# mihikamd/DP-GSAT

Hardware: AMD Instinct MI355X
Metric: million edges/s (attn+sample+aggregate fwd+bwd) (higher is better)
Workload: dtype f32

## Files before the change

dp_gsat_amd/_lib.py:

```python
from __future__ import annotations

import ctypes
import os
from ctypes import c_char_p, c_float, c_int, c_int32, c_int64, c_size_t, c_uint64, c_void_p

import torch

_HERE = os.path.dirname(os.path.abspath(__file__))
LIB_PATH = os.path.join(_HERE, "libgsat_hip.so")

P, I64, I32, F32, SZ, INT, U64 = c_void_p, c_int64, c_int32, c_float, c_size_t, c_int, c_uint64

SIGNATURES = {
    "gsat_abi_version": (INT, []),
    "gsat_seed_next": (INT, [P, P, P]),
    "gsat_last_error": (c_char_p, []),
    "gsat_csr_workspace_bytes": (SZ, [I64, I64]),
    "gsat_rev_workspace_bytes": (SZ, [I64]),
    "gsat_build_csr": (INT, [P, P, I64, I64, P, P, P, P, P, SZ, P]),
    "gsat_reverse_edge_perm": (INT, [P, I64, I64, P, P, P, SZ, P]),
    "gsat_reverse_edge_perm_csr": (INT, [P, P, P, P, P, P, P, P, I64, I64, P, P, P]),
    "gsat_segment_ptr": (INT, [P, I64, I64, P, P, P]),
    "gsat_gather_i64": (INT, [P, I64, P, I64, P, P]),
    "gsat_row_chunks_workspace_bytes": (SZ, [I64]),
    "gsat_row_chunks": (INT, [P, I64, P, P, SZ, P]),
    "gsat_long_row_partial_floats": (SZ, [I64, I64]),
    "gsat_aggr_sum_fwd": (INT, [P, P, P, P, P, P, P, I64, I64, I64, F32, P, P, P, P]),
    "gsat_aggr_sum_bwd": (INT, [P, P, P, P, P, P, P, I64, I64, I64, F32, P, P, P, P, P, P]),
    "gsat_pna_fwd": (INT, [P, P, P, P, P, P, I64, I64, P, INT, P, INT, F32, F32, P, P]),
    "gsat_pna_bwd": (INT, [P, P, P, P, P, P, P, I64, I64, P, INT, P, INT, F32, F32, P, P, P, P, P]),
    "gsat_pna_long_row_floats": (SZ, [I64, I64, INT]),
    "gsat_pna_fwd_long": (INT, [P, P, P, P, P, P, I64, I64, I64, P, INT, P, INT, F32, F32, P, P, P, P]),
    "gsat_pna_bwd_long": (INT, [P, P, P, P, P, P, P, I64, I64, I64, P, INT, P, INT, F32, F32, P, P, P, P, P, P, P]),
    "gsat_pna_tile_plan": (INT, [I64, I64, P, P, P]),
    "gsat_pna_build_tiles": (INT, [P, P, P, P, P, I64, INT, INT, INT, P, P, P, P]),
    "gsat_pna_bwd_tiled": (INT, [P, P, P, P, P, P, P, I64, INT, INT, INT, P, P, I64, I64, I64, P, INT, P, INT, P, P, P, P, P, P, P]),
    "gsat_pna_fwd_compact": (INT, [P, P, P, P, P, I64, I64, P, INT, P, P, P]),
    "gsat_pna_post_fwd": (INT, [P, P, P, I64, I64, INT, P, I64, P, I64, P, P]),
    "gsat_pna_post_dw_workspace_floats": (SZ, [I64, I64, INT, I64]),
    "gsat_pna_post_dw": (INT, [P, P, P, I64, I64, INT, P, I64, P, P, SZ, P]),
    "gsat_pna_fwd_node_att": (INT, [P, P, P, P, I64, I64, P, INT, P, INT, F32, F32, P, P]),
    "gsat_pna_bwd_tiled_node_att": (INT, [P, P, P, P, P, P, I64, INT, INT, INT, P, P, I64, I64, I64, P, INT, P, INT, P, P, P, P, P, P, P, INT, P]),
    "gsat_csr_pair_workspace_bytes": (SZ, [I64, I64]),
    "gsat_build_csr_pair": (INT, [P, I64, I64] + [P] * 12 + [P, SZ, P]),
    "gsat_segment_ptr32": (INT, [P, I64, I64, P, P, P, P]),
    "gsat_bn_workspace_floats": (SZ, [I64, I64]),
    "gsat_bn_fwd": (INT, [P, P, P, P, P, I64, I64, INT, F32, F32, INT, P, P, P, P, P]),
    "gsat_bn_bwd": (INT, [P, P, P, P, P, P, I64, I64, INT, INT, P, P, P, P, P]),
    "gsat_bn_act_fwd": (INT, [P, P, P, P, P, I64, I64, INT, F32, F32, INT, P, F32, U64, P, P, P, P, P, P]),
    "gsat_bn_act_bwd": (INT, [P, P, P, P, P, P, I64, I64, INT, INT, F32, U64, P, P, P, P, P, P, P]),
    "gsat_bn_local_sum": (INT, [P, P, I64, I64, P, P, P]),
    "gsat_bn_apply_fwd": (INT, [P, P, P, P, P, I64, I64, INT, P, F32, U64, P, P, P]),
    "gsat_bn_local_bwd_sums": (INT, [P, P, P, P, P, P, I64, I64, INT, F32, U64, P, P, P, P, P]),
    "gsat_bn_apply_bwd": (INT, [P, P, P, P, P, P, P, P, I64, P, I64, I64, INT, F32, U64, P, P, P, P]),
    "gsat_relu_dropout_fwd": (INT, [P, I64, I64, F32, U64, P, P, P]),
    "gsat_relu_dropout_bwd": (INT, [P, P, I64, I64, F32, P, P]),
    "gsat_colsum_workspace_floats": (SZ, [I64]),
    "gsat_colsum": (INT, [P, I64, I64, P, P, P]),
    "gsat_embsum_fwd": (INT, [P, P, INT, P, I64, I64, P, P]),
    "gsat_onehot_rows": (INT, [P, P, INT, I64, I64, P, P]),
    "gsat_gemm_workspace_floats": (SZ, [INT, I64, I64, I64]),
    "gsat_gemm_f32": (INT, [INT, INT, I64, I64, I64, P, I64, P, I64, P, I64, P, INT, P, SZ, P]),
    "gsat_gemm_bf16x3": (INT, [INT, INT, I64, I64, I64, P, I64, P, I64, P, I64, P, INT, P, SZ, P]),
    "gsat_attn_fwd_workspace_bytes": (SZ, [P]),
    "gsat_attn_fwd_kind": (I32, [P]),
    "gsat_attn_bwd_workspace_bytes": (SZ, [P]),
    "gsat_attn_fwd": (INT, [P, P]),
    "gsat_attn_bwd": (INT, [P, P, P]),
# ... 94 lines not shown
```

dp_gsat_amd/csrc/bookkeeping.hip:

```cpp
#include "common.h"
#include <rocprim/rocprim.hpp>

namespace gsat {

constexpr int64_t GSAT_COUNTING_MAX_KEYS = 1 << 20;

static thread_local char g_err[512] = {0};
void set_error(const char* fmt, ...) {
    va_list ap;
    va_start(ap, fmt);
    vsnprintf(g_err, sizeof(g_err), fmt, ap);
    va_end(ap);
}
const char* get_error() { return g_err; }

__global__ void k_seed_next(uint64_t* __restrict__ state, uint64_t* __restrict__ out) {
    const uint64_t c = state[1] + 1;
    state[1] = c;
    uint64_t z = state[0] + c * 0x9E3779B97F4A7C15ull;
    z = (z ^ (z >> 30)) * 0xBF58476D1CE4E5B9ull;
    z = (z ^ (z >> 27)) * 0x94D049BB133111EBull;
    z ^= z >> 31;
    out[0] = z & 0x7FFFFFFFFFFFFFFFull;
}
// ... 298 lines not shown
            if (k >= N) {
                const int c0 = (int32_t)(first[N] >> 32);
                rowptr_src[k - N] = beg - (int32_t)E;
                chunk_ptr_src[k - N] = chunks - c0;
                if (k == 2 * N) status[2] = chunks - c0;
            }
        } else {
            rowptr_dst[k] = beg;
        }
        if (k < R && (int32_t)first[k + 1] - beg > COUNT_ELEM_ROW)
            long_rows[atomicAdd(long_count, 1)] = (int32_t)k;
    }
    if (k < total) {
        const int r = rowkey[k];
        const int beg = (int32_t)first[r], end = (int32_t)first[r + 1];
        if (end - beg > COUNT_ELEM_ROW) return;
        const int v = slot[k];
        int rank = 0;
        for (int j = beg; j < end; ++j) rank += slot[j] < v;
        perm[beg + rank] = v;
    }
}

__global__ __launch_bounds__(COUNT_LONG_BLOCK) void k_pair_order_long(const int64_t* __restrict__ first, int32_t* __restrict__ slot,
                                                                       int32_t* __restrict__ perm, const int32_t* __restrict__ long_rows,
                                                                       const int32_t* __restrict__ long_count) {
    __shared__ int32_t buf[COUNT_CHUNK];
    const int nlong = *long_count;
    for (int q = blockIdx.x; q < nlong; q += gridDim.x) {
        const int k = long_rows[q];
        const int beg = (int32_t)first[k], end = (int32_t)first[k + 1], deg = end - beg;
        const int nchunks = (deg + COUNT_CHUNK - 1) / COUNT_CHUNK;
        for (int c = 0; c < nchunks; ++c) {
            const int cb = beg + c * COUNT_CHUNK, len = min(COUNT_CHUNK, end - cb);
            int p2 = 64;
            while (p2 < len) p2 <<= 1;
            for (int i = threadIdx.x; i < p2; i += COUNT_LONG_BLOCK) buf[i] = i < len ? slot[cb + i] : 0x7fffffff;
            __syncthreads();
            for (int size = 2; size <= p2; size <<= 1)
                for (int stride = size >> 1; stride > 0; stride >>= 1) {
                    for (int t = threadIdx.x; t < (p2 >> 1); t += COUNT_LONG_BLOCK) {
                        const int lo = 2 * t - (t & (stride - 1)), hi = lo + stride;
                        const bool up = (lo & size) == 0;
                        const int a = buf[lo], b = buf[hi];
                        if ((a > b) == up) { buf[lo] = b; buf[hi] = a; }
                    }
                    __syncthreads();
                }
            int32_t* outp = nchunks == 1 ? perm : slot;
            for (int i = threadIdx.x; i < len; i += COUNT_LONG_BLOCK) outp[cb + i] = buf[i];
            __syncthreads();
        }
        if (nchunks == 1) continue;
        for (int i = threadIdx.x; i < deg; i += COUNT_LONG_BLOCK) {
            const int v = slot[beg + i], own = i / COUNT_CHUNK;
            int r = i - own * COUNT_CHUNK;
            for (int c = 0; c < nchunks; ++c) {
                if (c == own) continue;
                const int32_t* base = slot + beg + c * COUNT_CHUNK;
                int lo = 0, hi = min(COUNT_CHUNK, deg - c * COUNT_CHUNK);
                while (lo < hi) {
                    const int mid = (lo + hi) >> 1;
                    if (base[mid] < v) lo = mid + 1; else hi = mid;
                }
                r += lo;
            }
            perm[beg + r] = v;
        }
        __syncthreads();
    }
}

struct CountAndChunks {
    const int32_t* cnt;
    __host__ __device__ int64_t operator()(int k) const {
        const int deg = cnt[k];
        const int64_t chunks = deg > GSAT_LONG_ROW_EDGES ? (deg + GSAT_LONG_ROW_EDGES - 1) / GSAT_LONG_ROW_EDGES : 0;
        return (int64_t)deg + (chunks << 32);
    }
};

static size_t count_scan_items_temp_bytes(int64_t items) {
    size_t tb = 0;
    auto in = rocprim::make_transform_iterator(rocprim::make_counting_iterator<int>(0), CountAndChunks{nullptr});
    int64_t* p = nullptr;
    (void)rocprim::exclusive_scan(nullptr, tb, in, p, (int64_t)0, (size_t)std::max<int64_t>(items, 1), rocprim::plus<int64_t>(), (hipStream_t)0);
    return align_up(tb, 256) + 256;
}
static size_t count_scan_temp_bytes(int64_t n) { return count_scan_items_temp_bytes(2 * n + 1); }

static bool counting_build(int64_t E) {
    static const int on = [] { const char* e = getenv("GSAT_CSR_COUNTING"); return e ? atoi(e) : 1; }();
    return on && 2 * E <= GSAT_COUNTING_MAX_KEYS;
}

// ... 7 lines not shown
        if (r >= num_rows) return 0;
        const int deg = rp[r + 1] - rp[r];
        return deg > GSAT_LONG_ROW_EDGES ? (deg + GSAT_LONG_ROW_EDGES - 1) / GSAT_LONG_ROW_EDGES : 0;
    }
};

__global__ void k_split_chunk_ptrs(const int32_t* __restrict__ scan, int64_t N, int32_t* __restrict__ chunk_ptr_dst,
                                   int32_t* __restrict__ chunk_ptr_src, int32_t* __restrict__ status) {
    int64_t i = (int64_t)blockIdx.x * blockDim.x + threadIdx.x;
    if (i > N) return;
    const int32_t d = scan[i], s = scan[N + 1 + i] - scan[N + 1];
    chunk_ptr_dst[i] = d;
    chunk_ptr_src[i] = s;
    if (i == N) { status[1] = d; status[2] = s; }
}

static size_t chunk2_scan_temp_bytes(int64_t n) {
    size_t tb = 0;
    auto in = rocprim::make_transform_iterator(rocprim::make_counting_iterator<int>(0), ChunkCount2{nullptr, nullptr, 0});
    int32_t* out = nullptr;
    (void)rocprim::exclusive_scan(nullptr, tb, in, out, 0, (size_t)(2 * n + 2), rocprim::plus<int>(), (hipStream_t)0);
    return align_up(tb, 256) + 256;
}

template <class K>
static size_t sort_temp_bytes(int64_t n) {
    size_t tb = 0;
    K* k = nullptr;
    int32_t* v = nullptr;
    (void)rocprim::radix_sort_pairs(nullptr, tb, k, k, v, v, (size_t)(n > 0 ? n : 1), 0, (unsigned)(8 * sizeof(K)), (hipStream_t)0);
    return align_up(tb, 256) + 256;
}

}

using namespace gsat;

extern "C" {

int gsat_abi_version(void) { return GSAT_ABI_VERSION; }

int gsat_seed_next(uint64_t* state, uint64_t* out, void* stream) {
    GSAT_REQUIRE(state && out, GSAT_ERR_ARG, "gsat_seed_next: null pointer");
    gsat::k_seed_next<<<1, 1, 0, (hipStream_t)stream>>>(state, out);
    GSAT_LAUNCH_CHECK();
    return GSAT_OK;
// ... 171 lines not shown
        GSAT_LAUNCH_CHECK();
        k_pair_order_long<<<256, COUNT_LONG_BLOCK, 0, stream>>>(first, slot, perm, long_rows, cnt + 2 * N + 1);
        GSAT_LAUNCH_CHECK();
    } else {
        GSAT_CHECK_HIP(gsat::zero_async(err_flag, 4 * sizeof(int32_t), stream));
        k_make_pair_keys<<<ceil_div(E, B), B, 0, stream>>>(edge_index, E, N, keys_in, ids, src32, dst32, err_flag);
        GSAT_LAUNCH_CHECK();
        const int end_bit = bits_for((uint64_t)(2 * N - 1));
        GSAT_CHECK_HIP(rocprim::radix_sort_pairs(temp, tb, keys_in, keys_out, ids, perm, (size_t)(2 * E), 0, (unsigned)end_bit, stream));
        k_pair_rowptrs<<<ceil_div(2 * N + 2, B), B, 0, stream>>>(keys_out, E, N, rowptr_dst, rowptr_src);
        GSAT_LAUNCH_CHECK();
    }
    k_pair_gather<<<ceil_div(2 * E, B), B, 0, stream>>>(edge_index, perm, E, N, rowptr_dst, src_by_dst, eid_by_dst, dst_by_src, eid_by_src,
                                                        slot_dst_of_srcslot);
    GSAT_LAUNCH_CHECK();
    if (counting) return GSAT_OK;
    auto in = rocprim::make_transform_iterator(rocprim::make_counting_iterator<int>(0), ChunkCount2{rowptr_dst, rowptr_src, (int)N});
    GSAT_CHECK_HIP(rocprim::exclusive_scan(temp2, tc, in, scan, 0, (size_t)(2 * N + 2), rocprim::plus<int>(), stream));
    k_split_chunk_ptrs<<<ceil_div(N + 1, B), B, 0, stream>>>(scan, N, chunk_ptr_dst, chunk_ptr_src, err_flag);
    GSAT_LAUNCH_CHECK();
    return GSAT_OK;
}

size_t gsat_row_chunks_workspace_bytes(int64_t num_rows) { return chunk_scan_temp_bytes(num_rows); }

int gsat_row_chunks(const int32_t* rowptr, int64_t num_rows, int32_t* chunk_ptr, void* workspace, size_t ws_bytes, void* stream_) {
    hipStream_t stream = (hipStream_t)stream_;
    GSAT_REQUIRE(num_rows >= 0 && num_rows < (1ll << 31) - 1 && rowptr && chunk_ptr, GSAT_ERR_ARG, "gsat_row_chunks: bad argument");
    size_t tb = chunk_scan_temp_bytes(num_rows);
    GSAT_REQUIRE(workspace && ws_bytes >= tb, GSAT_ERR_WORKSPACE, "gsat_row_chunks: workspace %zu < %zu", ws_bytes, tb);
    auto in = rocprim::make_transform_iterator(rocprim::make_counting_iterator<int>(0), ChunkCount{rowptr, (int)num_rows});
    GSAT_CHECK_HIP(rocprim::exclusive_scan(workspace, tb, in, chunk_ptr, 0, (size_t)(num_rows + 1), rocprim::plus<int>(), stream));
    return GSAT_OK;
}

int gsat_segment_ptr(const int64_t* seg_ids, int64_t n, int64_t num_seg, int32_t* ptr, int32_t* flags, void* stream_) {
    hipStream_t stream = (hipStream_t)stream_;
    GSAT_REQUIRE(n >= 0 && num_seg >= 0 && ptr && flags, GSAT_ERR_ARG, "gsat_segment_ptr: bad argument");
    GSAT_REQUIRE(n < (1ll << 31), GSAT_ERR_UNSUPPORTED, "gsat_segment_ptr: >2^31 rows");
    const int B = 256;
    GSAT_CHECK_HIP(gsat::zero_async(flags, sizeof(int32_t), stream));
    if (n > 0) {
        GSAT_REQUIRE(seg_ids, GSAT_ERR_ARG, "gsat_segment_ptr: null ids");
        k_check_sorted<<<ceil_div(n, B), B, 0, stream>>>(seg_ids, n, num_seg, flags);
        GSAT_LAUNCH_CHECK();
    }
// ... 28 lines not shown
```

dp_gsat_amd/csrc/common.h:

```cpp
#pragma once
#include <cstring>
#include <cstdint>
#include <cstdio>
#include <cstdarg>
#include <hip/hip_runtime.h>

#include "../../include/gsat_hip.h"

namespace gsat {

void set_error(const char* fmt, ...);
const char* get_error();

#define GSAT_CHECK_HIP(expr)                                                                  \
    do {                                                                                      \
        hipError_t _e = (expr);                                                               \
        if (_e != hipSuccess) {                                                               \
            gsat::set_error("%s:%d: %s -> %s", __FILE__, __LINE__, #expr, hipGetErrorString(_e)); \
            return GSAT_ERR_HIP;                                                              \
        }                                                                                     \
    } while (0)

#define GSAT_REQUIRE(cond, code, ...)                                                         \
    do {                                                                                      \
// ... 102 lines not shown
        c0 = n0; c1 = n1; c2 = n2; c3 = n3;
        k0 += 0x9E3779B9u; k1 += 0xBB67AE85u;
    }
    return make_uint4(c0, c1, c2, c3);
}

__device__ __forceinline__ float philox_noise_u(uint64_t seed, int row) {
    const uint4 r = philox4x32(seed, (uint32_t)row, 0u, 4u, 0x5A17u);
    return ((float)(r.x >> 9) + 0.5f) * (1.0f / 8388608.0f);
}

struct SeedRef {
    uint64_t value;
    const uint64_t* dev;
    __device__ __forceinline__ uint64_t get() const { return dev ? *dev : value; }
};

__device__ __forceinline__ float4 philox_keep4(uint64_t seed, int layer, int row, int c, float p) {
    uint4 r = philox4x32(seed, (uint32_t)row, (uint32_t)(c >> 2), (uint32_t)layer, 0x5A17u);
    const float k = 1.0f / 16777216.0f;
    return make_float4((float)(r.x >> 8) * k >= p ? 1.f : 0.f, (float)(r.y >> 8) * k >= p ? 1.f : 0.f,
                       (float)(r.z >> 8) * k >= p ? 1.f : 0.f, (float)(r.w >> 8) * k >= p ? 1.f : 0.f);
}
#endif

}
```

dp_gsat_amd/csrc/pna.hip:

```cpp
#include "common.h"
#include "pna_math.h"

namespace gsat {

constexpr int PNA_BLOCK = 128;
constexpr int SC_AMP = GSAT_SCALE_AMPLIFICATION, SC_ATT = GSAT_SCALE_ATTENUATION, SC_LIN = GSAT_SCALE_LINEAR, SC_INVLIN = GSAT_SCALE_INVERSE_LINEAR;

struct PnaCfg {
    int A, S;
    int aggr[8];
    int scal[8];
    float avg_lin, avg_log;
};

__device__ __forceinline__ int pna_xcd_remap(int b, int nb) {
    int q = nb >> 3, r = nb & 7, x = b & 7, i = b >> 3;
    return (x < r ? x * (q + 1) : r * (q + 1) + (x - r) * q) + i;
}

__device__ __forceinline__ float scaler_factor(int s, float deg, float avg_lin, float avg_log) {
    switch (s) {
        case SC_AMP: return logf(deg + 1.f) / avg_log;
        case SC_ATT: return deg == 0.f ? 1.f : avg_log / logf(deg + 1.f);
        case SC_LIN: return deg / avg_lin;
// ... 557 lines not shown
                        de.z = fmaf(Qe.z, w * ee.z, Pe.z) + (k == emin.z ? gmn_e.z : 0.f) + (k == emax.z ? gmx_e.z : 0.f);
                        de.w = fmaf(Qe.w, w * ee.w, Pe.w) + (k == emin.w ? gmn_e.w : 0.f) + (k == emax.w ? gmx_e.w : 0.f);
                        if (dedge) st4(dedge + (size_t)e * H + c, f4scale(w, de));
                        da += f4dot(de, ee);
                    }
                }
                if (datt) {
                    da = group_sum<LPR>(da);
                    if (lane == 0) datt[e] = c0 ? datt[e] + da : da;
                }
            }
        }
    }
}

constexpr int TILE_BLOCK = 512;

__global__ void k_pna_tiles(const int32_t* __restrict__ node_ptr, const int32_t* __restrict__ node_seg, const int32_t* __restrict__ rowptr,
                            const int32_t* __restrict__ rowptr_src, int N, int TN, int slack, int T, int4* __restrict__ desc,
                            int32_t* __restrict__ spill_count) {
    const int t = blockIdx.x * blockDim.x + threadIdx.x;
    if (t == 0 && spill_count) *spill_count = 0;
    if (t > T) return;
    const int64_t p = (int64_t)t * TN;
    int start = N;
    if (t < T && p < N) {
        start = (int)p;
        if (node_seg) {
            const int g0 = node_ptr[node_seg[p]];
            start = min((int)p, max(g0, (int)p - slack));
        }
    }
    desc[t] = make_int4(start, rowptr[start], rowptr_src[start], 0);
}

template <int LPR, int NAGG, bool NATT>
__global__ __launch_bounds__(TILE_BLOCK, 4) void k_pna_bwd_tile(
    const float* __restrict__ x, const float* __restrict__ att, const float* __restrict__ dout, const int32_t* __restrict__ rowptr,
    const int32_t* __restrict__ col, const int32_t* __restrict__ eid, const int4* __restrict__ desc,
    const int32_t* __restrict__ rowptr_src, const int32_t* __restrict__ slot_map, int H, int TE, int RCAP, float* dx,
    float* __restrict__ dmsg, float* datt, float* __restrict__ dw, const float* __restrict__ dx_add, int datt_acc) {
    constexpr int GPB = LaneGroups<LPR, TILE_BLOCK>::GPB;
    constexpr int RPW = 64 / LPR;
    constexpr int NSEG = NAGG * 2;
    extern __shared__ float4 smem4[];
    float4* erow = smem4;
    int* s_col = reinterpret_cast<int*>(erow + (size_t)TE * LPR);
    int* s_eid = s_col + TE;
    float* s_w = reinterpret_cast<float*>(s_eid);
    float* s_att = reinterpret_cast<float*>(s_eid + TE);
    int* s_slot = reinterpret_cast<int*>(s_att + TE);
    int* s_rp = s_slot + TE;
    int* s_rps = s_rp + RCAP + 1;
    float* s_na = reinterpret_cast<float*>(s_rps + RCAP + 1);
    float* s_dna = s_na + RCAP + 1;
    const int tid = threadIdx.x, wave = tid >> 6;
// ... 178 lines not shown
            acc.x += r.x; acc.y += r.y; acc.z += r.z; acc.w += r.w;
        }
        float sw = 0.f;
        for (int s_ = sb; s_ < se; ++s_) {
            const int kl = s_ < nsl ? s_slot[s_] : slot_map[s0 + s_] - k0;
            if (kl >= 0 && kl < ne) {
                const float4 v = erow[(size_t)kl * LPR + lane];
                acc.x += v.x; acc.y += v.y; acc.z += v.z; acc.w += v.w;
                if (NATT) sw += s_w[kl];
            }
        }
        st4(dx + (size_t)j * H + c, acc);
        if (NATT && datt && lane == 0) datt[j] = (s_dna[j - n0] + sw) + dprev;
    }
}

__global__ void k_pna_spill_rows(const int4* __restrict__ desc, int TN, int TE, const int32_t* __restrict__ rowptr_src,
                                 const int32_t* __restrict__ slot_map, int num_rows, int32_t* __restrict__ spill_rows,
                                 int32_t* __restrict__ spill_count) {
    const int j = blockIdx.x * blockDim.x + threadIdx.x;
    if (j >= num_rows) return;
    const int sb = rowptr_src[j], se = rowptr_src[j + 1];
    if (sb == se) return;
    int t = j / TN;
    if (j >= desc[t + 1].x) ++t;
    const int k0 = desc[t].y, ne = min(desc[t + 1].y - k0, TE);
    bool flag = false;
    for (int s_ = sb; s_ < se && !flag; ++s_) {
        const int k = slot_map[s_];
        flag = k < k0 || k >= k0 + ne;
    }
    if (flag) {
        const int idx = atomicAdd(spill_count, 1);
        if (idx < num_rows) spill_rows[idx] = j;
    }
}

template <int LPR>
__global__ __launch_bounds__(256) void k_pna_bwd_spill(const float* __restrict__ dmsg, const int4* __restrict__ desc, int TN, int TE,
                                                       const int32_t* __restrict__ rowptr_src, const int32_t* __restrict__ slot_map,
                                                       const int32_t* __restrict__ spill_rows, const int32_t* __restrict__ spill_count,
                                                       int num_rows, int H, float* __restrict__ dx, const float* __restrict__ dw,
                                                       float* __restrict__ dna) {
    const LaneGroups<LPR, 256> lg;
    constexpr int GPB = LaneGroups<LPR, 256>::GPB;
    const int lane = lg.lane, c = lane * 4;
    const int count = min(*spill_count, num_rows);
    if (lg.grp < 0) return;
    for (int i = blockIdx.x * GPB + lg.grp; i < count; i += gridDim.x * GPB) {
        const int j = spill_rows[i];
        const int sb = rowptr_src[j], se = rowptr_src[j + 1];
        int t = j / TN;
        if (j >= desc[t + 1].x) ++t;
        const int k0 = desc[t].y, ne = min(desc[t + 1].y - k0, TE);
// ... 325 lines not shown
```

dp_gsat_amd/graph_index.py:

```python
from __future__ import annotations

import os
from collections import OrderedDict
from typing import Optional

import torch

from . import _lib
from ._lib import call, ptr, stream


_SYNC_FREE = False
_VALIDATED: set = set()



_HUBS_SEEN = [False]
_STATUS_RING = []


def _harvest_status():
    bad = None
    for slot in _STATUS_RING:
        host, ev, owner = slot
# ... 30 lines not shown
    slot[2] = weakref.ref(index)
    index._status_event = slot[1]


_STRICT = False


def set_strict(flag: bool) -> None:
    global _STRICT
    _STRICT = bool(flag)


def strict() -> bool:
    return _STRICT


def set_sync_free(flag: bool) -> None:
    global _SYNC_FREE
    _SYNC_FREE = bool(flag)


def sync_free() -> bool:
    return _SYNC_FREE


def _i32(n, device):
    return torch.empty(max(int(n), 1), dtype=torch.int32, device=device)[: int(n)]


class BatchIndex:
    def __init__(self, edge_index: torch.Tensor, num_nodes: int):
        if edge_index.dim() != 2 or edge_index.shape[0] != 2 or edge_index.dtype != torch.int64:
            raise ValueError("edge_index must be an int64 tensor of shape [2, E]")
        _lib.load()
        if not edge_index.is_cuda:
            raise _lib.GsatHipError("BatchIndex needs a ROCm edge_index (no CPU fallback)")
        self._key_tensor = edge_index
        self.edge_index = edge_index.contiguous()
        self.N = int(num_nodes)
        self.E = int(edge_index.shape[1])
        self.device = edge_index.device
        dev = self.device
        E, N = self.E, self.N
        pair_build = os.environ.get("GSAT_CSR_PAIR", "1") != "0"
        self._err = (torch.empty if pair_build else torch.zeros)(8, dtype=torch.int32, device=dev)
        self._err3_fresh = True
# ... 6 lines not shown
         self.dst32) = (ints[i, :E] for i in range(7))
        if os.environ.get("GSAT_CSR_PAIR", "1") == "0":
            src, dst = self.edge_index[0], self.edge_index[1]
            wb = max(call_size("gsat_csr_workspace_bytes", E, N), 256)
            w1 = torch.empty(wb, dtype=torch.uint8, device=dev)
            call("gsat_build_csr", ptr(dst), ptr(src), E, N, ptr(self.rowptr_dst), ptr(self.src_by_dst), ptr(self.eid_by_dst),
                 ptr(self._err), ptr(w1), wb, stream())
            call("gsat_build_csr", ptr(src), ptr(dst), E, N, ptr(self.rowptr_src), ptr(self.dst_by_src), ptr(self.eid_by_src),
                 ptr(self._err), ptr(w1), wb, stream())
            cb = max(call_size("gsat_row_chunks_workspace_bytes", N), 256)
            w2 = torch.empty(cb, dtype=torch.uint8, device=dev)
            call("gsat_row_chunks", ptr(self.rowptr_dst), N, ptr(self.chunk_ptr_dst), ptr(w2), cb, stream())
            call("gsat_row_chunks", ptr(self.rowptr_src), N, ptr(self.chunk_ptr_src), ptr(w2), cb, stream())
            call("gsat_narrow_i64", ptr(src), E, ptr(self.src32), stream())
            call("gsat_narrow_i64", ptr(dst), E, ptr(self.dst32), stream())
            if E:
                inv = torch.empty(E, dtype=torch.int32, device=dev)
                inv[self.eid_by_dst.long()] = torch.arange(E, dtype=torch.int32, device=dev)
                self._slot_dst_of_srcslot.copy_(inv[self.eid_by_src.long()])
            self._partials, self._long, self._tiles = {}, None, {}
            self._checked, self._rev, self._rev_dev, self._rev_flags, self._undirected, self._graphs = False, None, None, None, None, {}
            self._long_async, self._status_queued, self._status_event = None, False, None
            return
        ws_bytes = max(call_size("gsat_csr_pair_workspace_bytes", E, N), 256)
        ws = torch.empty(ws_bytes, dtype=torch.uint8, device=dev)
        call("gsat_build_csr_pair", ptr(self.edge_index), E, N, ptr(self.rowptr_dst), ptr(self.src_by_dst), ptr(self.eid_by_dst),
             ptr(self.rowptr_src), ptr(self.dst_by_src), ptr(self.eid_by_src), ptr(self._slot_dst_of_srcslot),
             ptr(self.chunk_ptr_dst), ptr(self.chunk_ptr_src), ptr(self.src32), ptr(self.dst32), ptr(self._err), ptr(ws), ws_bytes,
             stream())
        self._partials = {}
        self._tiles = {}
        self._long = None
        self._checked = False
        self._rev = None
        self._rev_dev = None
        self._rev_flags = None
        self._undirected = None
        self._graphs = {}
        self._long_async = None
        self._status_queued, self._status_event = False, None
        if _SYNC_FREE:
            self._validate_once()

    @property
    def long_rows(self):
        if _SYNC_FREE and self._long is None:
            return (self.chunk_ptr_dst, self.chunk_ptr_src) if _HUBS_SEEN[0] else (None, None)
        if self._long is None or not self._checked:
            self._readback()
        return (self.chunk_ptr_dst if self._long[0] else None, self.chunk_ptr_src if self._long[1] else None)

    @property
    def long_rows_nowait(self):
        if _STRICT and not _SYNC_FREE and not self._checked and not torch.cuda.is_current_stream_capturing():
            self._readback()
        if self._long is not None:
            known = self._long
        else:
            if not _SYNC_FREE and not torch.cuda.is_current_stream_capturing():
                if not self._status_queued:
                    self._status_queued = True
                    _queue_status(self)
                elif self._long_async is None and self._status_event is not None and self._status_event.query():
                    _harvest_status()
            known = self._long_async
# ... 78 lines not shown
            if self._undirected is None:
                self._readback()
        return self._undirected

    @property
    def rev(self) -> Optional[torch.Tensor]:
        self.is_undirected
        return self._rev

    @property
    def slot_dst_of_srcslot(self) -> torch.Tensor:
        return self._slot_dst_of_srcslot

    def pna_tiles(self, H: int):
        import ctypes
        seg = next(iter(self._graphs.values())) if self._graphs else None
        key = (int(H), id(seg))
        hit = self._tiles.get(key)
        if hit is not None:
            return hit
        if H < 64:
            self._tiles[key] = False
            return False
        nominal, slack, ecap = ctypes.c_int32(), ctypes.c_int32(), ctypes.c_int32()
        budget = int(os.environ.get("GSAT_PNA_TILE_LDS", "0"))
        if _lib.load().gsat_pna_tile_plan(int(H), budget, ctypes.byref(nominal), ctypes.byref(slack), ctypes.byref(ecap)) != 0:
            self._tiles[key] = False
            return False
        T = (self.N + nominal.value - 1) // nominal.value
        tile_ptr = torch.empty(T + 1, 4, dtype=torch.int32, device=self.device)
        spill = torch.empty(self.N + 1, dtype=torch.int32, device=self.device)
        call("gsat_pna_build_tiles", ptr(seg.node_ptr) if seg is not None else None, ptr(seg.node_seg32) if seg is not None else None,
             ptr(self.rowptr_dst), ptr(self.rowptr_src), ptr(self._slot_dst_of_srcslot) if self.E else None, self.N, nominal.value,
             slack.value, ecap.value, ptr(tile_ptr), ptr(spill[1:]), ptr(spill[:1]), stream())
        out = (tile_ptr, T, nominal.value, nominal.value + slack.value, ecap.value, spill)
        self._tiles = {key: out}
        return out

    def graphs(self, batch: torch.Tensor, num_graphs: Optional[int] = None) -> "GraphSegments":
        key = (batch.data_ptr(), batch._version, int(batch.shape[0]))
        seg = self._graphs.get(key)
        if seg is None:
            if not self._err3_fresh:
                self._err[3:4].zero_()
            self._err3_fresh = False
            seg = GraphSegments(self, batch, num_graphs)
            self._graphs = {key: seg}
            self._checked = False
            if _SYNC_FREE:
                self._validate_once()
        return seg


class GraphSegments:

    def __init__(self, index: BatchIndex, batch: torch.Tensor, num_graphs: Optional[int] = None):
        if batch.dtype != torch.int64 or batch.dim() != 1:
            raise ValueError("batch must be an int64 vector")
        self.index = index
        self.batch = batch.contiguous()
        dev = batch.device
        n = int(batch.shape[0])
        if num_graphs is None:
            num_graphs = int(batch.max().item()) + 1 if n > 0 else 0
        self.G = int(num_graphs)
        self.node_ptr = torch.empty(self.G + 1, dtype=torch.int32, device=dev)
        flags = index._err[3:4]
        self.node_seg32 = _i32(n, dev)
        call("gsat_segment_ptr32", ptr(self.batch), n, self.G, ptr(self.node_ptr), ptr(self.node_seg32), ptr(flags), stream())
        self._flags = flags
        self._edge = None

    def check(self):
        self.index._checked = False
        self.index.check()

    @property
    def edge_segments(self):
        if self._edge is None:
            ix = self.index
            E, dev = ix.E, ix.device
            eg = torch.empty(max(E, 1), dtype=torch.int64, device=dev)[:E]
            call("gsat_gather_i64", ptr(self.batch), int(self.batch.shape[0]), ptr(ix.edge_index[0].contiguous()), E, ptr(eg), stream())
            ws_bytes = max(call_size("gsat_csr_workspace_bytes", E, self.G), 256)
            ws = torch.empty(ws_bytes, dtype=torch.uint8, device=dev)
            eptr = torch.empty(self.G + 1, dtype=torch.int32, device=dev)
            order = _i32(E, dev)
            err = torch.zeros(1, dtype=torch.int32, device=dev)
            call("gsat_build_csr", ptr(eg), None, E, self.G, ptr(eptr), None, ptr(order), ptr(err), ptr(ws), ws_bytes, stream())
            eg32 = _i32(E, dev)
            call("gsat_narrow_i64", ptr(eg), E, ptr(eg32), stream())
            self._edge = (eptr, order, eg, eg32)
# ... 29 lines not shown
```

include/gsat_hip.h:

```cpp
#ifndef GSAT_HIP_H
#define GSAT_HIP_H

#include <stddef.h>
#include <stdint.h>

#ifdef __cplusplus
extern "C" {
#endif

#define GSAT_ABI_VERSION 4

#define GSAT_OK 0
#define GSAT_ERR_HIP (-1)
#define GSAT_ERR_ARG (-2)
#define GSAT_ERR_WORKSPACE (-3)
#define GSAT_ERR_UNSUPPORTED (-4)
#define GSAT_ERR_BLAS (-5)

int gsat_abi_version(void);

int gsat_seed_next(uint64_t* state, uint64_t* out, void* stream);
const char* gsat_last_error(void);


// ... 3 lines not shown
int gsat_build_csr(const int64_t* rows, const int64_t* other, int64_t num_edges, int64_t num_rows,
                   int32_t* rowptr, int32_t* other_sorted, int32_t* perm, int32_t* err_flag,
                   void* workspace, size_t workspace_bytes, void* stream);

size_t gsat_csr_pair_workspace_bytes(int64_t E, int64_t num_nodes);
int gsat_build_csr_pair(const int64_t* edge_index, int64_t E, int64_t num_nodes, int32_t* rowptr_dst, int32_t* src_by_dst,
                        int32_t* eid_by_dst, int32_t* rowptr_src, int32_t* dst_by_src, int32_t* eid_by_src,
                        int32_t* slot_dst_of_srcslot, int32_t* chunk_ptr_dst, int32_t* chunk_ptr_src, int32_t* src32,
                        int32_t* dst32, int32_t* err_flag, void* workspace, size_t workspace_bytes, void* stream);

int gsat_reverse_edge_perm(const int64_t* edge_index, int64_t num_edges, int64_t num_nodes,
                           int32_t* rev, int32_t* flags, void* workspace, size_t workspace_bytes,
                           void* stream);

int gsat_reverse_edge_perm_csr(const int32_t* src32, const int32_t* dst32, const int32_t* rowptr_dst, const int32_t* src_by_dst,
                               const int32_t* eid_by_dst, const int32_t* rowptr_src, const int32_t* dst_by_src,
                               const int32_t* eid_by_src, int64_t num_edges, int64_t num_nodes, int32_t* rev, int32_t* flags,
                               void* stream);

int gsat_segment_ptr(const int64_t* seg_ids, int64_t num_rows, int64_t num_segments, int32_t* ptr,
                     int32_t* flags, void* stream);
int gsat_segment_ptr32(const int64_t* seg_ids, int64_t n, int64_t num_segments, int32_t* ptr, int32_t* seg_ids32,
                       int32_t* flags, void* stream);

int gsat_gather_i64(const int64_t* table, int64_t table_len, const int64_t* index, int64_t n, int64_t* out, void* stream);


#define GSAT_LONG_ROW_EDGES 256
size_t gsat_row_chunks_workspace_bytes(int64_t num_rows);
int gsat_row_chunks(const int32_t* rowptr, int64_t num_rows, int32_t* chunk_ptr ,
                    void* workspace, size_t workspace_bytes, void* stream);
size_t gsat_long_row_partial_floats(int64_t num_edges, int64_t H);

int gsat_aggr_sum_fwd(const float* x, const float* self_rows, const float* att, const float* edge_emb,
                      const int32_t* rowptr, const int32_t* col, const int32_t* eid,
                      int64_t num_rows, int64_t num_edges, int64_t H, float self_coef, float* out,
                      const int32_t* chunk_ptr, float* partial, void* stream);

int gsat_aggr_sum_bwd(const float* x, const float* att, const float* edge_emb, const float* dout,
                      const int32_t* rowptr_src, const int32_t* dst_sorted, const int32_t* eid_src,
                      int64_t num_rows, int64_t num_edges, int64_t H, float self_coef, float* dx, float* datt,
                      float* dedge_emb, const int32_t* chunk_ptr, float* partial, void* stream);


#define GSAT_AGG_SUM 0
#define GSAT_AGG_MEAN 1
// ... 230 lines not shown
```

Baseline: 125.6.

## Merge CSR pair build, batch segments and PNA tile plan into one fused index build

Adds a single batch-index build entry point that folds the CSR pair construction, the batch segment pointers and the PNA tile descriptors and spill detection into fewer multi-role kernels. Index construction is deferred lazily until the batch vector is known, so everything can be built in one pass. The goal is to cut kernel launches and repeated edge passes in per-batch bookkeeping. In exchange it adds lazy attribute machinery and a global tile-width heuristic, which makes the control flow more complex.

After: 126.4, median of 6. No clear change (+0.7%).

```diff
diff --git a/dp_gsat_amd/_lib.py b/dp_gsat_amd/_lib.py
--- a/dp_gsat_amd/_lib.py
+++ b/dp_gsat_amd/_lib.py
@@ -44,6 +44,8 @@
     "gsat_csr_pair_workspace_bytes": (SZ, [I64, I64]),
     "gsat_build_csr_pair": (INT, [P, I64, I64] + [P] * 12 + [P, SZ, P]),
     "gsat_segment_ptr32": (INT, [P, I64, I64, P, P, P, P]),
+    "gsat_batch_index_workspace_bytes": (SZ, [I64, I64]),
+    "gsat_build_batch_index": (INT, [P, I64, I64] + [P] * 12 + [P, I64, I64, P, P, INT, INT, INT, P, P, P, P, SZ, P]),
     "gsat_bn_workspace_floats": (SZ, [I64, I64]),
     "gsat_bn_fwd": (INT, [P, P, P, P, P, I64, I64, INT, F32, F32, INT, P, P, P, P, P]),
     "gsat_bn_bwd": (INT, [P, P, P, P, P, P, I64, I64, INT, INT, P, P, P, P, P]),
diff --git a/dp_gsat_amd/csrc/bookkeeping.hip b/dp_gsat_amd/csrc/bookkeeping.hip
--- a/dp_gsat_amd/csrc/bookkeeping.hip
+++ b/dp_gsat_amd/csrc/bookkeeping.hip
@@ -344,12 +344,9 @@
     }
 }
 
-__global__ __launch_bounds__(COUNT_LONG_BLOCK) void k_pair_order_long(const int64_t* __restrict__ first, int32_t* __restrict__ slot,
-                                                                       int32_t* __restrict__ perm, const int32_t* __restrict__ long_rows,
-                                                                       const int32_t* __restrict__ long_count) {
-    __shared__ int32_t buf[COUNT_CHUNK];
-    const int nlong = *long_count;
-    for (int q = blockIdx.x; q < nlong; q += gridDim.x) {
+__device__ __forceinline__ void order_long_rows(const int64_t* __restrict__ first, int32_t* __restrict__ slot, int32_t* __restrict__ perm,
+                                                const int32_t* __restrict__ long_rows, int nlong, int q0, int qstride, int32_t* buf) {
+    for (int q = q0; q < nlong; q += qstride) {
         const int k = long_rows[q];
         const int beg = (int32_t)first[k], end = (int32_t)first[k + 1], deg = end - beg;
         const int nchunks = (deg + COUNT_CHUNK - 1) / COUNT_CHUNK;
@@ -393,6 +390,13 @@
     }
 }
 
+__global__ __launch_bounds__(COUNT_LONG_BLOCK) void k_pair_order_long(const int64_t* __restrict__ first, int32_t* __restrict__ slot,
+                                                                       int32_t* __restrict__ perm, const int32_t* __restrict__ long_rows,
+                                                                       const int32_t* __restrict__ long_count) {
+    __shared__ int32_t buf[COUNT_CHUNK];
+    order_long_rows(first, slot, perm, long_rows, *long_count, blockIdx.x, gridDim.x, buf);
+}
+
 struct CountAndChunks {
     const int32_t* cnt;
     __host__ __device__ int64_t operator()(int k) const {
@@ -446,6 +450,151 @@
     (void)rocprim::exclusive_scan(nullptr, tb, in, out, 0, (size_t)(2 * n + 2), rocprim::plus<int>(), (hipStream_t)0);
     return align_up(tb, 256) + 256;
 }
+
+__global__ void k_index_prep(int32_t* __restrict__ cnt, int64_t ncnt, int32_t* __restrict__ status, int32_t* __restrict__ spill_count,
+                             const int64_t* __restrict__ ids, int64_t n, int64_t num_seg, int32_t* __restrict__ ids32,
+                             int32_t* __restrict__ ptr) {
+    const int64_t i = (int64_t)blockIdx.x * blockDim.x + threadIdx.x;
+    if (i < ncnt) cnt[i] = 0;
+    if (i < 4) status[i] = 0;
+    if (i == 0 && spill_count) *spill_count = 0;
+    if (!ptr) return;
+    if (i < n) {
+        const int64_t v = ids[i];
+        ids32[i] = (int32_t)(v < 0 ? 0 : (v >= num_seg ? num_seg - 1 : v));
+    }
+    if (i <= num_seg) {
+        int64_t lo = 0, hi = n;
+        while (lo < hi) {
+            int64_t mid = (lo + hi) >> 1;
+            if (ids[mid] < i) lo = mid + 1; else hi = mid;
+        }
+        ptr[i] = (int32_t)lo;
+    }
+}
+
+__global__ void k_pair_count_check(const int64_t* __restrict__ ei, int64_t E, int64_t N, int32_t* __restrict__ cnt,
+                                   int32_t* __restrict__ src32, int32_t* __restrict__ dst32, int32_t* status,
+                                   const int64_t* __restrict__ ids, int64_t n, int64_t num_seg) {
+    const int64_t e = (int64_t)blockIdx.x * blockDim.x + threadIdx.x;
+    if (e < E) {
+        int64_t s = ei[e], d = ei[E + e];
+        if (s < 0 || s >= N) { atomicAdd(status, 1); s = N - 1; }
+        if (d < 0 || d >= N) { atomicAdd(status, 1); d = N - 1; }
+        atomicAdd(&cnt[d], 1);
+        atomicAdd(&cnt[N + s], 1);
+        if (src32) src32[e] = (int32_t)s;
+        if (dst32) dst32[e] = (int32_t)d;
+    }
+    if (ids && e < n) {
+        const int64_t v = ids[e];
+        if (v < 0 || v >= num_seg || (e > 0 && ids[e - 1] > v)) atomicAdd(status + 3, 1);
+    }
+}
+
+__global__ void k_pair_place_ptrs(const int64_t* __restrict__ ei, int64_t E, int64_t N, const int64_t* __restrict__ first,
+                                  int32_t* __restrict__ cnt, int32_t* __restrict__ slot, int32_t* __restrict__ rowkey, int place_blocks,
+                                  int32_t* __restrict__ rowptr_dst, int32_t* __restrict__ rowptr_src, int32_t* __restrict__ chunk_ptr_dst,
+                                  int32_t* __restrict__ chunk_ptr_src, int32_t* __restrict__ status, int32_t* __restrict__ long_rows,
+                                  int32_t* __restrict__ long_count) {
+    if ((int)blockIdx.x >= place_blocks) {
+        const int64_t k = (int64_t)((int)blockIdx.x - place_blocks) * blockDim.x + threadIdx.x;
+        if (k > 2 * N) return;
+        const int64_t f = first[k];
+        const int beg = (int32_t)f, chunks = (int32_t)(f >> 32);
+        if (k <= N) { rowptr_dst[k] = beg; chunk_ptr_dst[k] = chunks; }
+        if (k == N) status[1] = chunks;
+        if (k >= N) {
+            const int c0 = (int32_t)(first[N] >> 32);
+            rowptr_src[k - N] = beg - (int32_t)E;
+            chunk_ptr_src[k - N] = chunks - c0;
+            if (k == 2 * N) status[2] = chunks - c0;
+        }
+        if (k < 2 * N && (int32_t)first[k + 1] - beg > COUNT_ELEM_ROW)
+            long_rows[atomicAdd(long_count, 1)] = (int32_t)k;
+        return;
+    }
+    int64_t e = (int64_t)blockIdx.x * blockDim.x + threadIdx.x;
+    if (e >= E) return;
+    int64_t s = ei[e], d = ei[E + e];
+    s = (s < 0 || s >= N) ? N - 1 : s;
+    d = (d < 0 || d >= N) ? N - 1 : d;
+    const int pd = (int32_t)first[d] + atomicSub(&cnt[d], 1) - 1, ps = (int32_t)first[N + s] + atomicSub(&cnt[N + s], 1) - 1;
+    slot[pd] = (int32_t)e; rowkey[pd] = (int32_t)d;
+    slot[ps] = (int32_t)e; rowkey[ps] = (int32_t)(N + s);
+}
+
+__global__ __launch_bounds__(COUNT_LONG_BLOCK) void k_pair_order_all(const int64_t* __restrict__ first, int64_t total, int32_t* slot,
+                                                                      const int32_t* __restrict__ rowkey, int32_t* __restrict__ perm,
+                                                                      int rank_blocks, const int32_t* __restrict__ long_rows,
+                                                                      const int32_t* __restrict__ long_count) {
+    __shared__ int32_t buf[COUNT_CHUNK];
+    if ((int)blockIdx.x >= rank_blocks) {
+        order_long_rows(first, slot, perm, long_rows, *long_count, (int)blockIdx.x - rank_blocks, (int)gridDim.x - rank_blocks, buf);
+        return;
+    }
+    const int64_t k = (int64_t)blockIdx.x * blockDim.x + threadIdx.x;
+    if (k >= total) return;
+    const int r = rowkey[k];
+    const int beg = (int32_t)first[r], end = (int32_t)first[r + 1];
+    if (end - beg > COUNT_ELEM_ROW) return;
+    const int v = slot[k];
+    int rank = 0;
+    for (int j = beg; j < end; ++j) rank += slot[j] < v;
+    perm[beg + rank] = v;
+}
+
+__global__ void k_pair_gather_spill(const int64_t* __restrict__ ei, const int32_t* __restrict__ perm, int64_t E, int64_t num_nodes,
+                                    const int32_t* __restrict__ rowptr_dst, int32_t* __restrict__ src_by_dst, int32_t* __restrict__ eid_by_dst,
+                                    int32_t* __restrict__ dst_by_src, int32_t* __restrict__ eid_by_src, int32_t* __restrict__ slot_dst_of_srcslot,
+                                    int gather_blocks, int spill_blocks, const int32_t* __restrict__ node_ptr,
+                                    const int32_t* __restrict__ node_seg, int4* __restrict__ desc, int TN, int slack, int T, int TE,
+                                    const int32_t* __restrict__ rowptr_src, int32_t* __restrict__ spill_rows,
+                                    int32_t* __restrict__ spill_count) {
+    auto clamp_id = [&](int64_t v) { return (int32_t)((v < 0 || v >= num_nodes) ? num_nodes - 1 : v); };
+    auto dst_slot = [&](int32_t e, int32_t d) {
+        int lo = rowptr_dst[d], hi = rowptr_dst[d + 1];
+        while (lo < hi) {
+            const int mid = (lo + hi) >> 1;
+            if (perm[mid] < e) lo = mid + 1; else hi = mid;
+        }
+        return lo;
+    };
+    auto desc_of = [&](int t) { return pna_tile_desc(t, node_ptr, node_seg, rowptr_dst, rowptr_src, (int)num_nodes, TN, slack, T); };
+    if ((int)blockIdx.x >= gather_blocks + spill_blocks) {
+        const int t = ((int)blockIdx.x - gather_blocks - spill_blocks) * blockDim.x + threadIdx.x;
+        if (t <= T) desc[t] = desc_of(t);
+        return;
+    }
+    if ((int)blockIdx.x >= gather_blocks) {
+        const int64_t j = (int64_t)((int)blockIdx.x - gather_blocks) * blockDim.x + threadIdx.x;
+        if (j >= num_nodes) return;
+        const int sb = rowptr_src[j], se = rowptr_src[j + 1];
+        if (sb == se) return;
+        const bool flag = pna_row_spills(desc_of, TN, TE, (int)j, sb, se, [&](int s_) {
+            const int32_t e = perm[E + s_];
+            return dst_slot(e, clamp_id(ei[E + e]));
+        });
+        if (flag) {
+            const int idx = atomicAdd(spill_count, 1);
+            if (idx < num_nodes) spill_rows[idx] = (int32_t)j;
+        }
+        return;
+    }
+    const int64_t k = (int64_t)blockIdx.x * blockDim.x + threadIdx.x;
+    if (k >= 2 * E) return;
+    const int32_t e = perm[k];
+    if (k < E) {
+        eid_by_dst[k] = e;
+        src_by_dst[k] = clamp_id(ei[e]);
+        return;
+    }
+    const int32_t d = clamp_id(ei[E + e]);
+    eid_by_src[k - E] = e;
+    dst_by_src[k - E] = d;
+    slot_dst_of_srcslot[k - E] = dst_slot(e, d);
+}
+
 
 template <class K>
 static size_t sort_temp_bytes(int64_t n) {
@@ -663,6 +812,88 @@
     return GSAT_OK;
 }
 
+size_t gsat_batch_index_workspace_bytes(int64_t E, int64_t N) { return gsat_csr_pair_workspace_bytes(E, N); }
+
+int gsat_build_batch_index(const int64_t* edge_index, int64_t E, int64_t N, int32_t* rowptr_dst, int32_t* src_by_dst, int32_t* eid_by_dst,
+                           int32_t* rowptr_src, int32_t* dst_by_src, int32_t* eid_by_src, int32_t* slot_dst_of_srcslot,
+                           int32_t* chunk_ptr_dst, int32_t* chunk_ptr_src, int32_t* src32, int32_t* dst32, int32_t* status,
+                           const int64_t* batch, int64_t batch_len, int64_t num_graphs, int32_t* node_ptr, int32_t* node_seg32,
+                           int rows_nominal, int rows_slack, int edges_cap, int32_t* tile_desc, int32_t* spill_rows, int32_t* spill_count,
+                           void* workspace, size_t ws_bytes, void* stream_) {
+    hipStream_t stream = (hipStream_t)stream_;
+    const bool with_batch = node_ptr != nullptr, with_tiles = tile_desc != nullptr;
+    GSAT_REQUIRE(E >= 0 && N >= 0 && rowptr_dst && rowptr_src && chunk_ptr_dst && chunk_ptr_src && status, GSAT_ERR_ARG,
+                 "gsat_build_batch_index: bad argument");
+    GSAT_REQUIRE(2 * E < (1ll << 31) && 2 * N + 2 < (1ll << 31), GSAT_ERR_UNSUPPORTED, "gsat_build_batch_index: >2^30 entries");
+    if (with_batch) {
+        GSAT_REQUIRE(batch_len >= 0 && batch_len < (1ll << 31) && num_graphs >= 0 && num_graphs < (1ll << 31) &&
+                     (batch_len == 0 || (batch && node_seg32)), GSAT_ERR_ARG, "gsat_build_batch_index: bad batch vector");
+    }
+    if (with_tiles) {
+        GSAT_REQUIRE(rows_nominal > 0 && rows_slack >= 0 && rows_slack <= rows_nominal && edges_cap > 0 && spill_rows && spill_count,
+                     GSAT_ERR_ARG, "gsat_build_batch_index: bad tile plan");
+        GSAT_REQUIRE(((uintptr_t)tile_desc & 15) == 0, GSAT_ERR_ARG, "gsat_build_batch_index: tile_desc must be 16-byte aligned");
+        GSAT_REQUIRE(!with_batch || batch_len == N, GSAT_ERR_ARG, "gsat_build_batch_index: windows need a batch vector of N entries");
+    }
+    const int32_t* seg_ptr = with_batch ? node_ptr : nullptr;
+    const int32_t* seg_ids = with_batch ? node_seg32 : nullptr;
+    if (E == 0 || !counting_build(E)) {
+        int rc = gsat_build_csr_pair(edge_index, E, N, rowptr_dst, src_by_dst, eid_by_dst, rowptr_src, dst_by_src, eid_by_src,
+                                     slot_dst_of_srcslot, chunk_ptr_dst, chunk_ptr_src, src32, dst32, status, workspace, ws_bytes, stream_);
+        if (rc != GSAT_OK) return rc;
+        if (with_batch) {
+            rc = gsat_segment_ptr32(batch, batch_len, num_graphs, node_ptr, node_seg32, status + 3, stream_);
+            if (rc != GSAT_OK) return rc;
+        }
+        if (with_tiles)
+            return gsat_pna_build_tiles(seg_ptr, seg_ids, rowptr_dst, rowptr_src, E ? slot_dst_of_srcslot : nullptr, N, rows_nominal,
+                                        rows_slack, edges_cap, tile_desc, spill_rows, spill_count, stream_);
+        return GSAT_OK;
+    }
+    GSAT_REQUIRE(edge_index && src_by_dst && eid_by_dst && dst_by_src && eid_by_src && slot_dst_of_srcslot && N > 0, GSAT_ERR_ARG,
+                 "gsat_build_batch_index: null pointer");
+    Arena ar(workspace, ws_bytes);
+    uint32_t* keys_in = ar.take<uint32_t>(2 * E);
+    uint32_t* keys_out = ar.take<uint32_t>(2 * E);
+    int32_t* slot = ar.take<int32_t>(2 * E);
+    int32_t* perm = ar.take<int32_t>(2 * E);
+    (void)ar.take<int32_t>(2 * N + 2);
+    int32_t* cnt = ar.take<int32_t>(2 * N + 2);
+    int64_t* first = ar.take<int64_t>(2 * N + 2);
+    size_t ts = count_scan_temp_bytes(N);
+    char* temp = ar.take<char>(std::max(sort_temp_bytes<uint32_t>(2 * E), ts));
+    GSAT_REQUIRE(ar.ok() && temp, GSAT_ERR_WORKSPACE, "gsat_build_batch_index: workspace %zu < %zu", ws_bytes, ar.off);
+    int32_t* long_rows = reinterpret_cast<int32_t*>(keys_in);
+    int32_t* rowkey = reinterpret_cast<int32_t*>(keys_out);
+    const int64_t nb = with_batch ? batch_len : 0, ng = with_batch ? num_graphs : 0;
+    const int64_t T = with_tiles ? ceil_div(N, rows_nominal) : 0;
+    const int B = 256;
+    k_index_prep<<<ceil_div(std::max<int64_t>(std::max<int64_t>(2 * N + 2, nb), ng + 1), B), B, 0, stream>>>(
+        cnt, 2 * N + 2, status, with_tiles ? spill_count : nullptr, with_batch ? batch : nullptr, nb, ng, node_seg32, node_ptr);
+    GSAT_LAUNCH_CHECK();
+    k_pair_count_check<<<ceil_div(std::max<int64_t>(E, nb), B), B, 0, stream>>>(edge_index, E, N, cnt, src32, dst32, status,
+                                                                               with_batch ? batch : nullptr, nb, ng);
+    GSAT_LAUNCH_CHECK();
+    auto cin = rocprim::make_transform_iterator(rocprim::make_counting_iterator<int>(0), CountAndChunks{cnt});
+    GSAT_CHECK_HIP(rocprim::exclusive_scan(temp, ts, cin, first, (int64_t)0, (size_t)(2 * N + 1), rocprim::plus<int64_t>(), stream));
+    const int place_blocks = (int)ceil_div(E, B);
+    k_pair_place_ptrs<<<place_blocks + (int)ceil_div(2 * N + 1, B), B, 0, stream>>>(edge_index, E, N, first, cnt, slot, rowkey, place_blocks,
+                                                                                    rowptr_dst, rowptr_src, chunk_ptr_dst, chunk_ptr_src,
+                                                                                    status, long_rows, cnt + 2 * N + 1);
+    GSAT_LAUNCH_CHECK();
+    const int rank_blocks = (int)ceil_div(2 * E, COUNT_LONG_BLOCK);
+    k_pair_order_all<<<rank_blocks + 256, COUNT_LONG_BLOCK, 0, stream>>>(first, 2 * E, slot, rowkey, perm, rank_blocks, long_rows,
+                                                                          cnt + 2 * N + 1);
+    GSAT_LAUNCH_CHECK();
+    const int gather_blocks = (int)ceil_div(2 * E, B), spill_blocks = with_tiles ? (int)ceil_div(N, B) : 0,
+              tile_blocks = with_tiles ? (int)ceil_div(T + 1, B) : 0;
+    k_pair_gather_spill<<<gather_blocks + spill_blocks + tile_blocks, B, 0, stream>>>(
+        edge_index, perm, E, N, rowptr_dst, src_by_dst, eid_by_dst, dst_by_src, eid_by_src, slot_dst_of_srcslot, gather_blocks, spill_blocks,
+        seg_ptr, seg_ids, (int4*)tile_desc, rows_nominal, seg_ids ? rows_slack : 0, (int)T, edges_cap, rowptr_src, spill_rows, spill_count);
+    GSAT_LAUNCH_CHECK();
+    return GSAT_OK;
+}
+
 size_t gsat_row_chunks_workspace_bytes(int64_t num_rows) { return chunk_scan_temp_bytes(num_rows); }
 
 int gsat_row_chunks(const int32_t* rowptr, int64_t num_rows, int32_t* chunk_ptr, void* workspace, size_t ws_bytes, void* stream_) {
diff --git a/dp_gsat_amd/csrc/common.h b/dp_gsat_amd/csrc/common.h
--- a/dp_gsat_amd/csrc/common.h
+++ b/dp_gsat_amd/csrc/common.h
@@ -148,6 +148,35 @@
     return make_float4((float)(r.x >> 8) * k >= p ? 1.f : 0.f, (float)(r.y >> 8) * k >= p ? 1.f : 0.f,
                        (float)(r.z >> 8) * k >= p ? 1.f : 0.f, (float)(r.w >> 8) * k >= p ? 1.f : 0.f);
 }
+
+__device__ __forceinline__ int4 pna_tile_desc(int t, const int32_t* __restrict__ node_ptr, const int32_t* __restrict__ node_seg,
+                                              const int32_t* __restrict__ rowptr, const int32_t* __restrict__ rowptr_src, int N, int TN,
+                                              int slack, int T) {
+    const int64_t p = (int64_t)t * TN;
+    int start = N;
+    if (t < T && p < N) {
+        start = (int)p;
+        if (node_seg) {
+            const int g0 = node_ptr[node_seg[p]];
+            start = min((int)p, max(g0, (int)p - slack));
+        }
+    }
+    return make_int4(start, rowptr[start], rowptr_src[start], 0);
+}
+
+template <class DescOf, class SlotOf>
+__device__ __forceinline__ bool pna_row_spills(DescOf desc_of, int TN, int TE, int j, int sb, int se, SlotOf slot_of) {
+    int t = j / TN;
+    int4 lo = desc_of(t), hi = desc_of(t + 1);
+    if (j >= hi.x) { lo = hi; hi = desc_of(t + 2); }
+    const int k0 = lo.y, ne = min(hi.y - k0, TE);
+    bool flag = false;
+    for (int s_ = sb; s_ < se && !flag; ++s_) {
+        const int k = slot_of(s_);
+        flag = k < k0 || k >= k0 + ne;
+    }
+    return flag;
+}
 #endif
 
 }
diff --git a/dp_gsat_amd/csrc/pna.hip b/dp_gsat_amd/csrc/pna.hip
--- a/dp_gsat_amd/csrc/pna.hip
+++ b/dp_gsat_amd/csrc/pna.hip
@@ -603,16 +603,7 @@
     const int t = blockIdx.x * blockDim.x + threadIdx.x;
     if (t == 0 && spill_count) *spill_count = 0;
     if (t > T) return;
-    const int64_t p = (int64_t)t * TN;
-    int start = N;
-    if (t < T && p < N) {
-        start = (int)p;
-        if (node_seg) {
-            const int g0 = node_ptr[node_seg[p]];
-            start = min((int)p, max(g0, (int)p - slack));
-        }
-    }
-    desc[t] = make_int4(start, rowptr[start], rowptr_src[start], 0);
+    desc[t] = pna_tile_desc(t, node_ptr, node_seg, rowptr, rowptr_src, N, TN, slack, T);
 }
 
 template <int LPR, int NAGG, bool NATT>
@@ -837,14 +828,7 @@
     if (j >= num_rows) return;
     const int sb = rowptr_src[j], se = rowptr_src[j + 1];
     if (sb == se) return;
-    int t = j / TN;
-    if (j >= desc[t + 1].x) ++t;
-    const int k0 = desc[t].y, ne = min(desc[t + 1].y - k0, TE);
-    bool flag = false;
-    for (int s_ = sb; s_ < se && !flag; ++s_) {
-        const int k = slot_map[s_];
-        flag = k < k0 || k >= k0 + ne;
-    }
+    const bool flag = pna_row_spills([&](int t) { return desc[t]; }, TN, TE, j, sb, se, [&](int s_) { return slot_map[s_]; });
     if (flag) {
         const int idx = atomicAdd(spill_count, 1);
         if (idx < num_rows) spill_rows[idx] = j;
diff --git a/dp_gsat_amd/graph_index.py b/dp_gsat_amd/graph_index.py
--- a/dp_gsat_amd/graph_index.py
+++ b/dp_gsat_amd/graph_index.py
@@ -76,6 +76,11 @@
 
 def sync_free() -> bool:
     return _SYNC_FREE
+
+
+_LAZY = ("rowptr_dst", "rowptr_src", "chunk_ptr_dst", "chunk_ptr_src", "src_by_dst", "eid_by_dst", "dst_by_src", "eid_by_src",
+         "_slot_dst_of_srcslot", "src32", "dst32", "_err")
+_TILE_WIDTH = [0]
 
 
 def _i32(n, device):
@@ -128,12 +133,6 @@
             self._checked, self._rev, self._rev_dev, self._rev_flags, self._undirected, self._graphs = False, None, None, None, None, {}
             self._long_async, self._status_queued, self._status_event = None, False, None
             return
-        ws_bytes = max(call_size("gsat_csr_pair_workspace_bytes", E, N), 256)
-        ws = torch.empty(ws_bytes, dtype=torch.uint8, device=dev)
-        call("gsat_build_csr_pair", ptr(self.edge_index), E, N, ptr(self.rowptr_dst), ptr(self.src_by_dst), ptr(self.eid_by_dst),
-             ptr(self.rowptr_src), ptr(self.dst_by_src), ptr(self.eid_by_src), ptr(self._slot_dst_of_srcslot),
-             ptr(self.chunk_ptr_dst), ptr(self.chunk_ptr_src), ptr(self.src32), ptr(self.dst32), ptr(self._err), ptr(ws), ws_bytes,
-             stream())
         self._partials = {}
         self._tiles = {}
         self._long = None
@@ -145,8 +144,54 @@
         self._graphs = {}
         self._long_async = None
         self._status_queued, self._status_event = False, None
-        if _SYNC_FREE:
+        if os.environ.get("GSAT_INDEX_MERGED", "1") == "0":
+            ws_bytes = max(call_size("gsat_csr_pair_workspace_bytes", E, N), 256)
+            ws = torch.empty(ws_bytes, dtype=torch.uint8, device=dev)
+            call("gsat_build_csr_pair", ptr(self.edge_index), E, N, ptr(self.rowptr_dst), ptr(self.src_by_dst), ptr(self.eid_by_dst),
+                 ptr(self.rowptr_src), ptr(self.dst_by_src), ptr(self.eid_by_src), ptr(self._slot_dst_of_srcslot),
+                 ptr(self.chunk_ptr_dst), ptr(self.chunk_ptr_src), ptr(self.src32), ptr(self.dst32), ptr(self._err), ptr(ws), ws_bytes,
+                 stream())
+            if _SYNC_FREE:
+                self._validate_once()
+            return
+        self._lazy = {name: self.__dict__.pop(name) for name in _LAZY}
+        self._built = False
+
+    def __getattr__(self, name):
+        if name in _LAZY and self.__dict__.get("_built") is False:
+            self._build(None, None)
+            return self.__dict__[name]
+        raise AttributeError(f"{type(self).__name__!r} object has no attribute {name!r}")
+
+    def _build(self, batch, num_graphs):
+        import ctypes
+        self.__dict__.update(self.__dict__.pop("_lazy"))
+        self._built = True
+        E, N, dev = self.E, self.N, self.device
+        seg = GraphSegments(self, batch, num_graphs, build=False) if batch is not None else None
+        H, tiles, tile_args = _TILE_WIDTH[0], None, (0, 0, 0, None, None, None)
+        if H >= 64 and seg is not None and int(batch.shape[0]) == N:
+            nominal, slack, ecap = ctypes.c_int32(), ctypes.c_int32(), ctypes.c_int32()
+            budget = int(os.environ.get("GSAT_PNA_TILE_LDS", "0"))
+            if _lib.load().gsat_pna_tile_plan(int(H), budget, ctypes.byref(nominal), ctypes.byref(slack), ctypes.byref(ecap)) == 0:
+                T = (N + nominal.value - 1) // nominal.value
+                tile_ptr = torch.empty(T + 1, 4, dtype=torch.int32, device=dev)
+                spill = torch.empty(N + 1, dtype=torch.int32, device=dev)
+                tiles = (tile_ptr, T, nominal.value, nominal.value + slack.value, ecap.value, spill)
+                tile_args = (nominal.value, slack.value, ecap.value, ptr(tile_ptr), ptr(spill[1:]), ptr(spill[:1]))
+        ws_bytes = max(call_size("gsat_batch_index_workspace_bytes", E, N), 256)
+        ws = torch.empty(ws_bytes, dtype=torch.uint8, device=dev)
+        call("gsat_build_batch_index", ptr(self.edge_index), E, N, ptr(self.rowptr_dst), ptr(self.src_by_dst), ptr(self.eid_by_dst),
+             ptr(self.rowptr_src), ptr(self.dst_by_src), ptr(self.eid_by_src), ptr(self._slot_dst_of_srcslot),
+             ptr(self.chunk_ptr_dst), ptr(self.chunk_ptr_src), ptr(self.src32), ptr(self.dst32), ptr(self._err),
+             ptr(seg.batch) if seg is not None else None, int(seg.batch.shape[0]) if seg is not None else 0, seg.G if seg is not None else 0,
+             ptr(seg.node_ptr) if seg is not None else None, ptr(seg.node_seg32) if seg is not None else None, *tile_args,
+             ptr(ws), ws_bytes, stream())
+        if tiles is not None:
+            self._tiles = {(int(H), id(seg)): tiles}
+        if seg is None and _SYNC_FREE:
             self._validate_once()
+        return seg
 
     @property
     def long_rows(self):
@@ -271,6 +316,7 @@
         if H < 64:
             self._tiles[key] = False
             return False
+        _TILE_WIDTH[0] = int(H)
         nominal, slack, ecap = ctypes.c_int32(), ctypes.c_int32(), ctypes.c_int32()
         budget = int(os.environ.get("GSAT_PNA_TILE_LDS", "0"))
         if _lib.load().gsat_pna_tile_plan(int(H), budget, ctypes.byref(nominal), ctypes.byref(slack), ctypes.byref(ecap)) != 0:
@@ -289,6 +335,13 @@
     def graphs(self, batch: torch.Tensor, num_graphs: Optional[int] = None) -> "GraphSegments":
         key = (batch.data_ptr(), batch._version, int(batch.shape[0]))
         seg = self._graphs.get(key)
+        if seg is None and self.__dict__.get("_built") is False:
+            GraphSegments.check_batch(batch)
+            seg = self._build(batch, num_graphs)
+            self._err3_fresh = False
+            self._graphs = {key: seg}
+            if _SYNC_FREE:
+                self._validate_once()
         if seg is None:
             if not self._err3_fresh:
                 self._err[3:4].zero_()
@@ -303,9 +356,13 @@
 
 class GraphSegments:
 
-    def __init__(self, index: BatchIndex, batch: torch.Tensor, num_graphs: Optional[int] = None):
+    @staticmethod
+    def check_batch(batch):
         if batch.dtype != torch.int64 or batch.dim() != 1:
             raise ValueError("batch must be an int64 vector")
+
+    def __init__(self, index: BatchIndex, batch: torch.Tensor, num_graphs: Optional[int] = None, build: bool = True):
+        self.check_batch(batch)
         self.index = index
         self.batch = batch.contiguous()
         dev = batch.device
@@ -316,7 +373,8 @@
         self.node_ptr = torch.empty(self.G + 1, dtype=torch.int32, device=dev)
         flags = index._err[3:4]
         self.node_seg32 = _i32(n, dev)
-        call("gsat_segment_ptr32", ptr(self.batch), n, self.G, ptr(self.node_ptr), ptr(self.node_seg32), ptr(flags), stream())
+        if build:
+            call("gsat_segment_ptr32", ptr(self.batch), n, self.G, ptr(self.node_ptr), ptr(self.node_seg32), ptr(flags), stream())
         self._flags = flags
         self._edge = None
 
diff --git a/include/gsat_hip.h b/include/gsat_hip.h
--- a/include/gsat_hip.h
+++ b/include/gsat_hip.h
@@ -49,6 +49,15 @@
                      int32_t* flags, void* stream);
 int gsat_segment_ptr32(const int64_t* seg_ids, int64_t n, int64_t num_segments, int32_t* ptr, int32_t* seg_ids32,
                        int32_t* flags, void* stream);
+
+size_t gsat_batch_index_workspace_bytes(int64_t E, int64_t num_nodes);
+int gsat_build_batch_index(const int64_t* edge_index, int64_t E, int64_t num_nodes, int32_t* rowptr_dst, int32_t* src_by_dst,
+                           int32_t* eid_by_dst, int32_t* rowptr_src, int32_t* dst_by_src, int32_t* eid_by_src,
+                           int32_t* slot_dst_of_srcslot, int32_t* chunk_ptr_dst, int32_t* chunk_ptr_src, int32_t* src32,
+                           int32_t* dst32, int32_t* status, const int64_t* batch, int64_t batch_len, int64_t num_graphs,
+                           int32_t* node_ptr, int32_t* node_seg32, int rows_nominal, int rows_slack, int edges_cap,
+                           int32_t* tile_desc, int32_t* spill_rows, int32_t* spill_count, void* workspace, size_t workspace_bytes,
+                           void* stream);
 
 int gsat_gather_i64(const int64_t* table, int64_t table_len, const int64_t* index, int64_t n, int64_t* out, void* stream);
 
```
